# ruc-aimc-lab/GeoFormer

Measured on NVIDIA B200. Metric: pairs_per_sec_640x480, higher is better.
Workload: dtype tf32 / fp16 tensor-core operands with fp32 accumulation (fp32 residual stream, fp16 intermediates), split-fp16 similarity, f16 backbone activations

## Files before the change

### geoformer_b200/_lib.py

```python
from __future__ import annotations

import ctypes
import os
from ctypes import c_char_p, c_float, c_int, c_int64, c_void_p

HERE = os.path.dirname(os.path.abspath(__file__))
LIB_PATH = os.path.join(HERE, "libgeoformer_sm100.so")

P, I, L, F = c_void_p, c_int, c_int64, c_float

SIGNATURES = {
    "gf_abi_version": (I, []),
    "gf_last_error": (c_char_p, []),
    "gf_init": (I, [I]),
    "gf_launch_count": (L, []),
    "gf_linear_tf32": (I, [P, P, P, P, L, I, I, I, I, I, P, P, I, P, P, P, P, P]),
    "gf_linear_ref": (I, [P, P, P, P, L, I, I, I, I, I, P, P, I, P, P, P, P, P]),
    "gf_conv3x3_f16": (I, [P, P, P, P, P, I, I, I, I, I, I, I, P]),
    "gf_conv_f16": (I, [P, P, P, P, P, I, I, I, I, I, I, I, I, I, P]),
    "gf_stem_conv7x7_f16": (I, [P, P, P, P, I, I, I, P]),
    "gf_upsample_add_f16": (I, [P, P, P, I, I, I, I, I, I, P]),
    "gf_conv_ref": (I, [P, P, P, P, P, I, I, I, I, I, I, I, I, P]),
    "gf_upsample_add_ref": (I, [P, P, P, I, I, I, I, I, I, P]),
    "gf_add_posenc": (I, [P, P, P, I, L, I, P]),
    "gf_linattn_partial_floats": (L, [I, I, I, I]),
    "gf_linear_mixed": (I, [P, P, P, P, I, I, L, I, I, I, I, I, P, P, I, P, P, P, P, P]),
    "gf_fine_layer": (I, [P, P, P, P, P, P, P, P, L, P]),
    "gf_linattn_reduce_f16": (I, [P, I, P, I, I, I, I, I, P, P, P, P]),
    "gf_linattn_apply_f16": (I, [P, I, P, P, P, I, I, I, I, I, P]),
    "gf_linattn_window_f16": (I, [P, I, P, I, P, I, P, L, I, I, I, P]),
    "gf_linattn_reduce": (I, [P, I, P, I, I, I, I, I, P, P, P, P]),
    "gf_linattn_apply": (I, [P, I, P, P, P, I, I, I, I, I, P]),
    "gf_linattn_window": (I, [P, I, P, I, P, I, P, L, I, I, I, P]),
    "gf_full_attention": (I, [P, I, P, I, P, I, P, I, I, I, I, I, P]),
    "gf_dense_kv_h16": (I, [P, I, P, I, I, I, I, I, I, P, P, P, P]),
    "gf_full_attention_tc": (I, [P, I, P, P, P, P, I, I, I, I, I, I, P]),
    "gf_full_attention_window": (I, [P, I, P, I, P, I, P, L, I, I, I, P]),
    "gf_full_attention_window_f16": (I, [P, I, P, I, P, I, P, L, I, I, I, P]),
    "gf_pack_split_f16": (I, [P, P, L, I, F, I, P]),
    "gf_similarity_f16x3": (I, [P, P, P, I, I, I, I, F, P]),
    "gf_similarity_ref": (I, [P, P, P, I, I, I, I, F, F, P]),
    "gf_dual_softmax_workspace_floats": (L, [I, I, I]),
    "gf_dual_softmax_stats": (I, [P, I, I, I, P, P, P, P, P, P]),
    "gf_dual_softmax_conf": (I, [P, I, I, I, P, P, P, P, P, P, P]),
    "gf_conf_row_col_max": (I, [P, I, I, I, P, P, P]),
    "gf_mnn_select": (I, [P, I, I, I, F, I, I, I, I, I, P, P, P, P, P]),
    "gf_coarse_match_fused_workspace_bytes": (L, [I, I, I]),
    "gf_coarse_match_fused": (I, [P, P, I, I, I, I, F, F, I, I, I, I, I, P, P, P, P]),
    "gf_coarse_match_fused_pass": (I, [P, P, I, I, I, I, F, P, I, P]),
    "gf_compact_coarse": (I, [P, P, I, I, I, I, F, P, P, P, P, P, P, P, P, L, P]),
# ... 72 lines not shown
```

### geoformer_b200/csrc/fine_layer.cu

```cuda
#include "common.cuh"
#include "ptx.cuh"

#include <cuda_fp16.h>

#include <atomic>
#include <cstdlib>

namespace gf {
extern std::atomic<int64_t> g_launches;

namespace fl {
constexpr int C = 128, TOK = 25, WIN = 5, ROWS = TOK * WIN, HEADS = 8, D = 16;
constexpr int BLK = 16384;
constexpr int NBLK = 30;
constexpr int STAGES = 3;
constexpr int R1 = 0, R2 = 65536, R3 = 131072;
constexpr int R3_BYTES = 32768;
constexpr int RING = R3 + R3_BYTES;
constexpr int BARS = RING + STAGES * BLK;
constexpr int LNX = BARS + 256;
constexpr int SMEM_BYTES = LNX + 8192 + 1024;
constexpr int EPI_WARPS = 16, THREADS = 64 + 32 * EPI_WARPS;
constexpr int D0 = 0, D1 = 384, D2 = 0, D3 = 384;

struct Params {
  const float* x;
  float* y;
  const float* gamma1; const float* beta1; const float* gamma2; const float* beta2;
  int64_t rows;
  int tiles;
  int cross;
  int debug;
};

__device__ __forceinline__ float ex2f(float x) { float y; asm("ex2.approx.ftz.f32 %0, %1;" : "=f"(y) : "f"(x)); return y; }
__device__ __forceinline__ float elu_plus1(float v) { return v > 0.f ? v + 1.f : ex2f(v * 1.4426950408889634f); }
__device__ __forceinline__ uint32_t pack2(float a, float b) {
  const __half2 h = __floats2half2_rn(a, b);
  return *reinterpret_cast<const uint32_t*>(&h);
}
__device__ __forceinline__ void epi_sync() { asm volatile("bar.sync 1, 512;" ::: "memory"); }

__device__ __forceinline__ void ldsm_x4(uint32_t (&r)[4], uint32_t addr) {
  asm volatile("ldmatrix.sync.aligned.m8n8.x4.shared.b16 {%0, %1, %2, %3}, [%4];"
               : "=r"(r[0]), "=r"(r[1]), "=r"(r[2]), "=r"(r[3]) : "r"(addr));
}
__device__ __forceinline__ void ldsm_x4_trans(uint32_t (&r)[4], uint32_t addr) {
  asm volatile("ldmatrix.sync.aligned.m8n8.x4.trans.shared.b16 {%0, %1, %2, %3}, [%4];"
               : "=r"(r[0]), "=r"(r[1]), "=r"(r[2]), "=r"(r[3]) : "r"(addr));
}
__device__ __forceinline__ void mma16816(float (&d)[4], const uint32_t (&a)[4], uint32_t b0, uint32_t b1) {
  asm volatile("mma.sync.aligned.m16n8k16.row.col.f32.f16.f16.f32 {%0, %1, %2, %3}, {%4, %5, %6, %7}, {%8, %9}, {%0, %1, %2, %3};"
               : "+f"(d[0]), "+f"(d[1]), "+f"(d[2]), "+f"(d[3]) : "r"(a[0]), "r"(a[1]), "r"(a[2]), "r"(a[3]), "r"(b0), "r"(b1));
}

__device__ __forceinline__ void row_stats32(const float (&v)[32], float2* lnx, int part, int r, float& mean, float& rstd) {
  float s = 0.f, ss = 0.f;
#pragma unroll
  for (int j = 0; j < 32; ++j) { s += v[j]; ss = fmaf(v[j], v[j], ss); }
  lnx[part * 128 + r] = make_float2(s, ss);
  epi_sync();
  const float2 p0 = lnx[r], p1 = lnx[128 + r], p2 = lnx[256 + r], p3 = lnx[384 + r];
  const float ts = (p0.x + p1.x) + (p2.x + p3.x), tss = (p0.y + p1.y) + (p2.y + p3.y);
  mean = ts * (1.f / 128.f);
  const float var = fmaxf(tss * (1.f / 128.f) - mean * mean, 0.f);
  rstd = rsqrtf(var + 1e-5f);
}
__device__ __forceinline__ void normalize32(float (&v)[32], float mean, float rstd, const float* __restrict__ gamma,
                                            const float* __restrict__ beta) {
#pragma unroll
  for (int j = 0; j < 8; ++j) {
    const float4 g4 = __ldg(reinterpret_cast<const float4*>(gamma) + j);
    const float4 b4 = __ldg(reinterpret_cast<const float4*>(beta) + j);
    v[4 * j] = (v[4 * j] - mean) * rstd * g4.x + b4.x;
    v[4 * j + 1] = (v[4 * j + 1] - mean) * rstd * g4.y + b4.y;
    v[4 * j + 2] = (v[4 * j + 2] - mean) * rstd * g4.z + b4.z;
    v[4 * j + 3] = (v[4 * j + 3] - mean) * rstd * g4.w + b4.w;
  }
}
__device__ __forceinline__ void warp_arrive(uint64_t* bar, int lane) {
  ptx::fence_proxy_async();
  ptx::tc_fence_before();
  __syncwarp();
  if (lane == 0) ptx::mbar_arrive(bar);
}

__global__ void __launch_bounds__(THREADS, 1)
fine_layer_kernel(const __grid_constant__ CUtensorMap tmX, const __grid_constant__ CUtensorMap tmS,
                  const __grid_constant__ CUtensorMap tmW, const Params p) {
  extern __shared__ uint8_t smem_raw[];
  uint8_t* smem = reinterpret_cast<uint8_t*>((reinterpret_cast<uintptr_t>(smem_raw) + 1023) & ~uintptr_t(1023));
  uint64_t* full_bar = reinterpret_cast<uint64_t*>(smem + BARS);
  uint64_t* empty_bar = full_bar + STAGES;
  uint64_t* x_full = empty_bar + STAGES;
  uint64_t* s_full = x_full + 1;
  uint64_t* d_full = s_full + 1;
  uint64_t* a_full = d_full + 4;
  uint64_t* d0_free = a_full + 3;
  uint64_t* r1_free = d0_free + 1;
  uint64_t* r2_free = r1_free + 1;
  uint32_t* tmem_slot = reinterpret_cast<uint32_t*>(r2_free + 1);

  const int warp = threadIdx.x >> 5, lane = threadIdx.x & 31;

  if (warp == 0 && lane == 0) { ptx::prefetch_tmap(&tmX); ptx::prefetch_tmap(&tmS); ptx::prefetch_tmap(&tmW); }
  if (warp == 1) {
    if (lane == 0) {
      for (int i = 0; i < STAGES; ++i) { ptx::mbar_init(&full_bar[i], 1); ptx::mbar_init(&empty_bar[i], 1); }
      ptx::mbar_init(x_full, 1);
      ptx::mbar_init(s_full, 1);
      for (int i = 0; i < 4; ++i) ptx::mbar_init(&d_full[i], 1);
      for (int i = 0; i < 3; ++i) ptx::mbar_init(&a_full[i], EPI_WARPS);
      ptx::mbar_init(d0_free, 1);
      ptx::mbar_init(r1_free, 1);
      ptx::mbar_init(r2_free, 1);
      ptx::fence_barrier_init();
    }
    __syncwarp();
    ptx::tmem_alloc(tmem_slot, 512);
  }
  ptx::tc_fence_before();
  __syncthreads();
  ptx::tc_fence_after();
  const uint32_t tmem_base = *tmem_slot;

  if (warp == 0) {
    if (lane == 0) {
      int stage = 0; uint32_t phase = 0;
      auto weights = [&](int b0, int b1) {
        for (int b = b0; b < b1; ++b) {
          ptx::mbar_wait(&empty_bar[stage], phase ^ 1);
          ptx::mbar_expect_tx(&full_bar[stage], BLK);
          ptx::tma_load_3d(smem + RING + stage * BLK, &tmW, &full_bar[stage], 0, b * 128, 0);
          if (++stage == STAGES) { stage = 0; phase ^= 1; }
        }
      };
      auto load_x = [&](int t) {
        ptx::mbar_expect_tx(x_full, 4 * BLK);
        for (int kb = 0; kb < 4; ++kb) ptx::tma_load_3d(smem + R1 + kb * BLK, &tmX, x_full, kb * 32, t * ROWS, 0);
      };
      auto load_src = [&](int t) {
        ptx::mbar_expect_tx(s_full, 4 * BLK);
        for (int kb = 0; kb < 4; ++kb) ptx::tma_load_3d(smem + R2 + kb * BLK, &tmS, s_full, kb * 32, t * ROWS, 0);
      };
      load_x(blockIdx.x);
      if (p.cross) load_src(blockIdx.x);
      weights(0, 12);
      int it = 0;
      for (int t = blockIdx.x; t < p.tiles; t += gridDim.x, ++it) {
        const int tn = t + gridDim.x;
        const bool next = tn < p.tiles;
        weights(12, 20);
        if (next) { ptx::mbar_wait(r1_free, it & 1); load_x(tn); }
        weights(20, 30);
        if (next) {
          weights(0, 4);
          if (p.cross) { ptx::mbar_wait(r2_free, it & 1); load_src(tn); }
          weights(4, 12);
        }
      }
    }
  } else if (warp == 1) {
    {
      constexpr uint32_t id_tf32 = ptx::umma_idesc(2, 128, 128);
      constexpr uint32_t id_f16 = ptx::umma_idesc(0, 128, 128);
      const uint32_t smem0 = __shfl_sync(0xffffffffu, ptx::smem_addr(smem), 0);
      const uint32_t tb = __shfl_sync(0xffffffffu, tmem_base, 0);
      const uint32_t s_r1 = smem0 + R1, s_r2 = smem0 + R2, s_r3 = smem0 + R3, s_ring = smem0 + RING;
      const uint32_t bar0 = smem0 + BARS;
      auto bar_addr = [&](const uint64_t* b) -> uint32_t { return bar0 + (uint32_t)((const uint8_t*)b - (const uint8_t*)full_bar); };
      int stage = 0; uint32_t phase = 0;
      auto step = [&](int kind, uint32_t a_addr, uint32_t d_col, bool first) {
        ptx::mbar_wait(&full_bar[stage], phase);
        ptx::tc_fence_after();
        const uint32_t a_lo = ptx::umma_desc_lo(a_addr), b_lo = ptx::umma_desc_lo(s_ring + stage * BLK);
        if (ptx::elect_one()) {
          if (kind == 0) {
#pragma unroll
            for (int k = 0; k < 4; ++k) ptx::umma_lo<0>(tb + d_col, a_lo + 2 * k, b_lo + 2 * k, ptx::kDescHiSw128, id_tf32, (first && k == 0) ? 0u : 1u);
          } else {
#pragma unroll
            for (int k = 0; k < 4; ++k) ptx::umma_lo<1>(tb + d_col, a_lo + 2 * k, b_lo + 2 * k, ptx::kDescHiSw128, id_f16, (first && k == 0) ? 0u : 1u);
          }
          ptx::umma_commit_addr(bar_addr(&empty_bar[stage]));
        }
        if (++stage == STAGES) { stage = 0; phase ^= 1; }
      };
      auto commit = [&](const uint64_t* b) { if (ptx::elect_one()) ptx::umma_commit_addr(bar_addr(b)); };
      auto gemm0 = [&](int i) {
        ptx::mbar_wait(x_full, i & 1);
        ptx::tc_fence_after();
        for (int kb = 0; kb < 4; ++kb) step(0, s_r1 + kb * BLK, D0, kb == 0);
        if (p.cross) { ptx::mbar_wait(s_full, i & 1); ptx::tc_fence_after(); }
        const uint32_t a0 = p.cross ? s_r2 : s_r1;
        for (int nc = 1; nc < 3; ++nc)
          for (int kb = 0; kb < 4; ++kb) step(0, a0 + kb * BLK, D0 + nc * 128, kb == 0);
        commit(&d_full[0]);
      };
      gemm0(0);
      int it = 0;
      for (int t = blockIdx.x; t < p.tiles; t += gridDim.x, ++it) {
        const uint32_t par = it & 1;
        ptx::mbar_wait(d0_free, par);
        ptx::tc_fence_after();
        for (int nc = 0; nc < 2; ++nc)
          for (int kb = 0; kb < 4; ++kb) step(0, s_r1 + kb * BLK, D2 + nc * 128, kb == 0);
        commit(r1_free);
        ptx::mbar_wait(&a_full[0], par);
        ptx::tc_fence_after();
        for (int kb = 0; kb < 2; ++kb) step(1, s_r3 + kb * BLK, D1, kb == 0);
        commit(&d_full[1]);
        ptx::mbar_wait(&a_full[1], par);
        ptx::tc_fence_after();
        for (int nc = 0; nc < 2; ++nc)
          for (int kb = 0; kb < 2; ++kb) step(1, s_r2 + 2 * BLK + kb * BLK, D2 + nc * 128, false);
        commit(&d_full[2]);
        ptx::mbar_wait(&a_full[2], par);
        ptx::tc_fence_after();
        for (int kb = 0; kb < 4; ++kb) step(1, s_r2 + kb * BLK, D3, kb == 0);
        commit(&d_full[3]);
        commit(r2_free);
        if (t + (int)gridDim.x < p.tiles) gemm0(it + 1);
      }
    }
  } else {
    const int quad = warp & 3;
    const int part = (warp - 2) >> 2;
    const int r = quad * 32 + lane;
    const int et = threadIdx.x - 64;
    const int ew = warp - 2;
    const uint32_t t_lane = tmem_base + (uint32_t(quad * 32) << 16);
    uint8_t* r2 = smem + R2;
    uint8_t* r3 = smem + R3;
    float2* lnx = reinterpret_cast<float2*>(smem + LNX);
    const int sw7 = r & 7;
    const int g = lane >> 2, tq = lane & 3;
    const int lrow = lane & 7, lmat = lane >> 3;
    int it = 0;
    for (int t = blockIdx.x; t < p.tiles; t += gridDim.x, ++it) {
      const uint32_t par = it & 1;
      const int64_t row0 = (int64_t)t * ROWS;
      ptx::mbar_wait(&d_full[0], par);
      ptx::tc_fence_after();
      {
        float va[32], vb[32];
        ptx::tmem_ld_32x32(t_lane + D0 + 32 * part, va);
        ptx::tmem_ld_wait();
        ptx::tmem_ld_32x32(t_lane + D0 + 32 * (4 + part), vb);
        uint4 u[4];
#pragma unroll
        for (int j = 0; j < 32; ++j) va[j] = elu_plus1(va[j]);
#pragma unroll
        for (int j = 0; j < 4; ++j) {
          u[j].x = pack2(va[8 * j], va[8 * j + 1]); u[j].y = pack2(va[8 * j + 2], va[8 * j + 3]);
          u[j].z = pack2(va[8 * j + 4], va[8 * j + 5]); u[j].w = pack2(va[8 * j + 6], va[8 * j + 7]);
        }
        {
          uint8_t* dst = r3 + (part >> 1) * BLK + r * 128;
#pragma unroll
          for (int j = 0; j < 4; ++j) *reinterpret_cast<uint4*>(dst + ((((part & 1) * 4 + j) ^ sw7) << 4)) = u[j];
        }
        ptx::tmem_ld_wait();
        ptx::tmem_ld_32x32(t_lane + D0 + 32 * (8 + part), va);
#pragma unroll
        for (int j = 0; j < 32; ++j) vb[j] = elu_plus1(vb[j]);
#pragma unroll
        for (int j = 0; j < 4; ++j) {
          u[j].x = pack2(vb[8 * j], vb[8 * j + 1]); u[j].y = pack2(vb[8 * j + 2], vb[8 * j + 3]);
          u[j].z = pack2(vb[8 * j + 4], vb[8 * j + 5]); u[j].w = pack2(vb[8 * j + 6], vb[8 * j + 7]);
        }
        {
          uint8_t* dst = r2 + r * 256;
#pragma unroll
          for (int j = 0; j < 4; ++j) *reinterpret_cast<uint4*>(dst + (((part * 4 + j) ^ (r & 15)) << 4)) = u[j];
        }
        ptx::tmem_ld_wait();
#pragma unroll
        for (int j = 0; j < 4; ++j) {
          u[j].x = pack2(va[8 * j], va[8 * j + 1]); u[j].y = pack2(va[8 * j + 2], va[8 * j + 3]);
          u[j].z = pack2(va[8 * j + 4], va[8 * j + 5]); u[j].w = pack2(va[8 * j + 6], va[8 * j + 7]);
        }
        {
          uint8_t* dst = r2 + 32768 + r * 256;
#pragma unroll
          for (int j = 0; j < 4; ++j) *reinterpret_cast<uint4*>(dst + (((part * 4 + j) ^ (r & 15)) << 4)) = u[j];
        }
      }
      ptx::tc_fence_before();
      epi_sync();
      if (et == 0) ptx::mbar_arrive(d0_free);
      if (!(p.debug & 2)) {
        const uint32_t k16 = ptx::smem_addr(r2), v16 = k16 + 32768, q16 = ptx::smem_addr(r3);
#pragma unroll 1
        for (int pair = ew; pair < WIN * HEADS; pair += EPI_WARPS) {
          const int w = pair >> 3, h = pair & 7;
          float cv[2][4] = {{0.f, 0.f, 0.f, 0.f}, {0.f, 0.f, 0.f, 0.f}}, co[2][4] = {{0.f, 0.f, 0.f, 0.f}, {0.f, 0.f, 0.f, 0.f}};
#pragma unroll
          for (int ks = 0; ks < 2; ++ks) {
            const int tok0 = TOK * w + 16 * ks;
            uint32_t a[4], b[4];
            const int wlast = TOK * w + TOK - 1;
            const int arow = min(tok0 + lrow + ((lmat >> 1) << 3), wlast), achunk = 2 * h + (lmat & 1);
            ldsm_x4_trans(a, v16 + arow * 256 + ((achunk ^ (arow & 15)) << 4));
            const int brow = min(tok0 + lrow + ((lmat & 1) << 3), wlast), bchunk = 2 * h + (lmat >> 1);
            ldsm_x4_trans(b, k16 + brow * 256 + ((bchunk ^ (brow & 15)) << 4));
            uint32_t o0 = (g == 0) ? 0x3C003C00u : 0u, o2 = o0;
            if (ks == 1) {
              if (tq == 0) { a[2] &= 0xFFFFu; a[3] &= 0xFFFFu; o2 &= 0xFFFFu; } else { a[2] = 0u; a[3] = 0u; o2 = 0u; }
            }
            const uint32_t ao[4] = {o0, 0u, o2, 0u};
            mma16816(cv[0], a, b[0], b[1]); mma16816(cv[1], a, b[2], b[3]);
            mma16816(co[0], ao, b[0], b[1]); mma16816(co[1], ao, b[2], b[3]);
          }
// ... 5 lines not shown
            const int tok0 = TOK * w + 16 * mt;
            uint32_t aq[4];
            const int qrow = min(tok0 + lrow + ((lmat & 1) << 3), TOK * w + TOK - 1), qchunk = (h & 3) * 2 + (lmat >> 1);
            ldsm_x4(aq, q16 + (h >> 2) * BLK + qrow * 128 + ((qchunk ^ (qrow & 7)) << 4));
            float o0[4] = {0.f, 0.f, 0.f, 0.f}, o1[4] = {0.f, 0.f, 0.f, 0.f}, dn[4] = {0.f, 0.f, 0.f, 0.f};
            mma16816(o0, aq, bq[0][0], bq[0][1]);
            mma16816(o1, aq, bq[1][0], bq[1][1]);
            mma16816(dn, aq, bq[2][0], bq[2][1]);
            const float z_lo = 1.f / (__shfl_sync(0xffffffffu, dn[0], lane & ~3) + 1e-6f);
            const float z_hi = 1.f / (__shfl_sync(0xffffffffu, dn[2], lane & ~3) + 1e-6f);
            const int row_lo = tok0 + g, row_hi = row_lo + 8;
            __syncwarp();
            uint8_t* blk = r3 + (h >> 2) * BLK;
            const int c0 = (h & 3) * 2;
            *reinterpret_cast<uint32_t*>(blk + row_lo * 128 + ((c0 ^ (row_lo & 7)) << 4) + 4 * tq) = pack2(o0[0] * z_lo, o0[1] * z_lo);
            *reinterpret_cast<uint32_t*>(blk + row_lo * 128 + (((c0 + 1) ^ (row_lo & 7)) << 4) + 4 * tq) = pack2(o1[0] * z_lo, o1[1] * z_lo);
            if (mt == 0 || g == 0) {
              *reinterpret_cast<uint32_t*>(blk + row_hi * 128 + ((c0 ^ (row_hi & 7)) << 4) + 4 * tq) = pack2(o0[2] * z_hi, o0[3] * z_hi);
              *reinterpret_cast<uint32_t*>(blk + row_hi * 128 + (((c0 + 1) ^ (row_hi & 7)) << 4) + 4 * tq) = pack2(o1[2] * z_hi, o1[3] * z_hi);
            }
          }
        }
      }
      warp_arrive(&a_full[0], lane);
      ptx::mbar_wait(&d_full[1], par);
      ptx::tc_fence_after();
      {
        float v[32];
        ptx::tmem_ld_32x32(t_lane + D1 + 32 * part, v);
        ptx::tmem_ld_wait();
        float mean, rstd;
        row_stats32(v, lnx, part, r, mean, rstd);
        if (!(p.debug & 4)) {
          normalize32(v, mean, rstd, p.gamma1 + 32 * part, p.beta1 + 32 * part);
          uint8_t* dst = r2 + 2 * BLK + (part >> 1) * BLK + r * 128;
#pragma unroll
          for (int j = 0; j < 4; ++j) {
            uint4 u;
            u.x = pack2(v[8 * j], v[8 * j + 1]); u.y = pack2(v[8 * j + 2], v[8 * j + 3]);
            u.z = pack2(v[8 * j + 4], v[8 * j + 5]); u.w = pack2(v[8 * j + 6], v[8 * j + 7]);
            *reinterpret_cast<uint4*>(dst + ((((part & 1) * 4 + j) ^ sw7) << 4)) = u;
          }
        }
      }
      warp_arrive(&a_full[1], lane);
      ptx::mbar_wait(&d_full[2], par);
      ptx::tc_fence_after();
      {
        float va[32], vb[32];
        ptx::tmem_ld_32x32(t_lane + D2 + 32 * part, va);
        ptx::tmem_ld_32x32(t_lane + D2 + 32 * (4 + part), vb);
        ptx::tmem_ld_wait();
        if (!(p.debug & 4)) {
#pragma unroll
          for (int q = 0; q < 2; ++q) {
            const int c = part + 4 * q;
            const float* v = q ? vb : va;
            uint8_t* dst = r2 + (c >> 1) * BLK + r * 128;
#pragma unroll
            for (int j = 0; j < 4; ++j) {
              uint4 u;
              u.x = pack2(fmaxf(v[8 * j], 0.f), fmaxf(v[8 * j + 1], 0.f)); u.y = pack2(fmaxf(v[8 * j + 2], 0.f), fmaxf(v[8 * j + 3], 0.f));
              u.z = pack2(fmaxf(v[8 * j + 4], 0.f), fmaxf(v[8 * j + 5], 0.f)); u.w = pack2(fmaxf(v[8 * j + 6], 0.f), fmaxf(v[8 * j + 7], 0.f));
              *reinterpret_cast<uint4*>(dst + ((((c & 1) * 4 + j) ^ sw7) << 4)) = u;
            }
          }
        }
      }
      warp_arrive(&a_full[2], lane);
      uint8_t* box = r3 + ew * 2048;
      const int64_t grow0 = row0 + quad * 32;
      const int trow = lane >> 2, tch = lane & 3;
      float4 xr[4];
#pragma unroll
      for (int i = 0; i < 4; ++i) {
        const int rr = 8 * i + trow;
        xr[i] = make_float4(0.f, 0.f, 0.f, 0.f);
        if (quad * 32 + rr < ROWS && grow0 + rr < p.rows)
          xr[i] = __ldg(reinterpret_cast<const float4*>(p.x + (grow0 + rr) * C + 32 * part) + tch);
      }
      ptx::mbar_wait(&d_full[3], par);
      ptx::tc_fence_after();
      {
        float v[32];
        ptx::tmem_ld_32x32(t_lane + D3 + 32 * part, v);
        ptx::tmem_ld_wait();
        ptx::tc_fence_before();
        float mean, rstd;
        row_stats32(v, lnx + 512, part, r, mean, rstd);
        if (!(p.debug & 4)) {
          normalize32(v, mean, rstd, p.gamma2 + 32 * part, p.beta2 + 32 * part);
#pragma unroll
          for (int c = 0; c < 2; ++c) {
#pragma unroll
            for (int j = 0; j < 4; ++j)
              *reinterpret_cast<float4*>(box + lane * 64 + ((j ^ ((lane >> 1) & 3)) << 4)) =
                  make_float4(v[16 * c + 4 * j], v[16 * c + 4 * j + 1], v[16 * c + 4 * j + 2], v[16 * c + 4 * j + 3]);
            __syncwarp();
            float4 xn[4];
#pragma unroll
            for (int i = 0; i < 4; ++i) {
              const int rr = 8 * i + trow;
              const bool live = quad * 32 + rr < ROWS && grow0 + rr < p.rows;
              if (c == 0) {
                xn[i] = make_float4(0.f, 0.f, 0.f, 0.f);
                if (live) xn[i] = __ldg(reinterpret_cast<const float4*>(p.x + (grow0 + rr) * C + 32 * part + 16) + tch);
              }
              const float4 y4 = *reinterpret_cast<const float4*>(box + rr * 64 + ((tch ^ ((rr >> 1) & 3)) << 4));
              if (live)
                *(reinterpret_cast<float4*>(p.y + (grow0 + rr) * C + 32 * part + 16 * c) + tch) =
                    make_float4(y4.x + xr[i].x, y4.y + xr[i].y, y4.z + xr[i].z, y4.w + xr[i].w);
            }
            if (c == 0) {
#pragma unroll
              for (int i = 0; i < 4; ++i) xr[i] = xn[i];
            }
            __syncwarp();
          }
        }
      }
      epi_sync();
    }
  }

  ptx::tc_fence_before();
  __syncthreads();
  if (warp == 1) {
    ptx::tc_fence_after();
    ptx::tmem_dealloc(tmem_base, 512);
  }
}

}
}

using namespace gf;

extern "C" int gf_fine_layer(const float* x, const float* src, const void* wpack, const float* gamma1, const float* beta1,
                             const float* gamma2, const float* beta2, float* y, int64_t windows, gf_stream_t stream) {
  if (windows < 0 || !x || !src || !wpack || !y || y == x || y == src) return gf_set_error(GF_ERR_ARG, "gf_fine_layer: bad arguments");
  if (windows == 0) return GF_OK;
  const int64_t rows = windows * fl::TOK;
  if (rows > 0x7fffff00LL) return gf_set_error(GF_ERR_ARG, "gf_fine_layer: too many rows");
  CUtensorMap tx, ts, tw;
  int rc;
  if ((rc = make_tmap(&tx, x, 4, fl::C, rows, 1, fl::C, 0, 128))) return rc;
  if ((rc = make_tmap(&ts, src, 4, fl::C, rows, 1, fl::C, 0, 128))) return rc;
  if ((rc = make_tmap(&tw, wpack, 4, 32, (int64_t)fl::NBLK * 128, 1, 32, 0, 128))) return rc;
  fl::Params p{};
  p.x = x; p.y = y; p.gamma1 = gamma1; p.beta1 = beta1; p.gamma2 = gamma2; p.beta2 = beta2;
  p.rows = rows; p.tiles = (int)((windows + fl::WIN - 1) / fl::WIN); p.cross = (src != x) ? 1 : 0;
  { const char* dbg = getenv("GF_FL_DEBUG"); p.debug = dbg ? atoi(dbg) : 0; }
  GF_SMEM_OPTIN(fl::fine_layer_kernel, fl::SMEM_BYTES);
  const int grid = p.tiles < num_sms() ? p.tiles : num_sms();
  fl::fine_layer_kernel<<<grid, fl::THREADS, fl::SMEM_BYTES, (cudaStream_t)stream>>>(tx, ts, tw, p);
  g_launches++;
  GF_CHECK_LAUNCH();
  return GF_OK;
}
```

### geoformer_b200/ops.py

```python
from __future__ import annotations

import os
import threading
from typing import Optional, Tuple

import torch

from . import _lib

EPI_RELU, EPI_TANH, EPI_ELU1, EPI_LN = 1, 2, 4, 8

_LINEAR_IMPL = "tf32"
_SIM_IMPL = "f16x3"
_ATTN_IMPL = "tf32"
_ACT16 = os.environ.get("GF_ACT16", "1") != "0"


def act16() -> bool:
    return _ACT16 and _LINEAR_IMPL == "tf32"


def set_precision(linear: Optional[str] = None, similarity: Optional[str] = None,
                  attention: Optional[str] = None, activations: Optional[str] = None) -> None:
    global _LINEAR_IMPL, _SIM_IMPL, _ATTN_IMPL, _ACT16
# ... 308 lines not shown
    _call("gf_full_attention", q.data_ptr(), ldq, k.data_ptr(), ldk, v.data_ptr(), ldv, out.data_ptr(), n, l, s, heads, dim,
          _stream())
    return out


def full_attention_window(q: torch.Tensor, ldq: int, k: torch.Tensor, ldk: int, v: torch.Tensor, ldv: int, n_windows: int,
                          tokens: int, heads: int, dim: int) -> torch.Tensor:
    assert q.dtype == k.dtype == v.dtype
    out = torch.empty((n_windows * tokens, heads * dim), device=q.device, dtype=torch.float32)
    _call("gf_full_attention_window" + ("_f16" if q.dtype == torch.float16 else ""), q.data_ptr(), ldq, k.data_ptr(), ldk,
          v.data_ptr(), ldv, out.data_ptr(), n_windows, tokens, heads, dim, _stream())
    return out


def fine_layer_fused(x: torch.Tensor, src: torch.Tensor, wpack: torch.Tensor, n1w, n1b, n2w, n2b) -> torch.Tensor:
    _chk(x); _chk(src)
    m, t, c = x.shape
    assert (t, c) == (25, 128) and src.shape == x.shape and x.is_contiguous() and src.is_contiguous()
    assert wpack.dtype == torch.uint8 and wpack.shape == (30, 128, 128) and wpack.is_contiguous()
    y = torch.empty_like(x)
    _call("gf_fine_layer", x.data_ptr(), src.data_ptr(), wpack.data_ptr(), n1w.data_ptr(), n1b.data_ptr(), n2w.data_ptr(),
          n2b.data_ptr(), y.data_ptr(), m, _stream(), tag="[cross]" if src.data_ptr() != x.data_ptr() else "[self]")
    return y


def similarity(f0: torch.Tensor, f1: torch.Tensor, temperature: float, impl: Optional[str] = None) -> torch.Tensor:
    _chk(f0); _chk(f1)
    n, l, c = f0.shape
    s = f1.shape[1]
    assert f0.is_contiguous() and f1.is_contiguous()
    sim = torch.empty((n, l, s), device=f0.device, dtype=torch.float32)
    in_scale = 1.0 / c ** 0.5
    if (impl or _SIM_IMPL) == "f16x3":
        a3 = torch.empty((n, l, 3 * c), device=f0.device, dtype=torch.float16)
        b3 = torch.empty((n, s, 3 * c), device=f0.device, dtype=torch.float16)
        _call("gf_pack_split_f16", f0.data_ptr(), a3.data_ptr(), n * l, c, in_scale, 0, _stream())
        _call("gf_pack_split_f16", f1.data_ptr(), b3.data_ptr(), n * s, c, in_scale, 1, _stream())
        _call("gf_similarity_f16x3", a3.data_ptr(), b3.data_ptr(), sim.data_ptr(), n, l, s, 3 * c,
              1.0 / temperature, _stream())
    else:
        _call("gf_similarity_ref", f0.data_ptr(), f1.data_ptr(), sim.data_ptr(), n, l, s, c, in_scale,
                  1.0 / temperature, _stream())
    return sim


def dual_softmax_(sim: torch.Tensor) -> Tuple[torch.Tensor, torch.Tensor, torch.Tensor]:
# ... 212 lines not shown
```

### include/geoformer_b200.h

```cpp
#ifndef GEOFORMER_B200_H_
#define GEOFORMER_B200_H_

#include <stdint.h>

#ifdef __cplusplus
extern "C" {
#endif

#define GF_ABI_VERSION 1

#define GF_OK 0
#define GF_ERR_ARG (-1)
#define GF_ERR_LAUNCH (-2)
#define GF_ERR_DRIVER (-3)
#define GF_ERR_DEVICE (-4)

#define GF_EPI_RELU 1
#define GF_EPI_TANH 2
#define GF_EPI_ELU1 4
#define GF_EPI_LN 8

typedef void* gf_stream_t;

int gf_abi_version(void);
// ... 90 lines not shown
                        gf_stream_t stream);
int gf_masked_softmax_rows(float* x, int heads, int n, int l, int s_pad, const int* cnt_per_sample, gf_stream_t stream);
int gf_gather_anchor_kv_f16(const float* q, int ldq, const float* k, int ldk, const float* v, int ldv, int n, int l,
                            int heads, int dim, const int* anchor_idx, const int* anchor_cnt, int anchor_cap, int s_pad,
                            void* q16, void* kg, void* vt, gf_stream_t stream);
int gf_gather_anchor_kv_h16(const void* k, int ldk, const void* v, int ldv, int n, int l, int heads, int dim,
                            const int* anchor_idx, const int* anchor_cnt, int anchor_cap, int s_pad, void* kg, void* vt,
                            gf_stream_t stream);
int gf_geo_self_attention_tc(const void* q16, int ldq, const void* kg, const void* vt, float* out, int n, int l,
                             int heads, int dim, int s_pad, const int* anchor_cnt, gf_stream_t stream);
int gf_gemm_tf32_batched(const float* A, int64_t lda, int64_t a_batch_stride, const float* B, int64_t ldb,
                         int64_t b_batch_stride, float* Y, int64_t ldy, int64_t y_batch_stride, int M, int N, int K,
                         int batches, float out_scale, gf_stream_t stream);

int gf_geo_cross_attention(const float* q, int ldq, const float* kproj, int ldk, const float* vproj, int ldv,
                           float* out, int n, int l, int s, int heads, int dim, const int* widx, int window2,
                           gf_stream_t stream);
int gf_geo_cross_attention_f16(const void* q, int ldq, const void* kproj, int ldk, const void* vproj, int ldv, void* out,
                               int n, int l, int s, int heads, int dim, const int* widx, int window2, gf_stream_t stream);
int gf_select_rows(float* dst, const float* src, const int* flag, int n, int64_t l, int c, gf_stream_t stream);

int gf_fine_layer(const float* x, const float* src, const void* wpack, const float* gamma1, const float* beta1,
                  const float* gamma2, const float* beta2, float* y, int64_t windows, gf_stream_t stream);
int gf_fine_gather(const float* fine_nhwc, int hf, int wf, int c, const int64_t* b_ids, const int64_t* tok_ids,
                   int64_t m, int wc, int stride, int window, float* out, gf_stream_t stream);
int gf_fine_gather_f16(const void* fine_nhwc, int hf, int wf, int c, const int64_t* b_ids, const int64_t* tok_ids,
                        int64_t m, int wc, int stride, int window, float* out, gf_stream_t stream);
int gf_fine_gather_f16_f16(const void* fine_nhwc, int hf, int wf, int c, const int64_t* b_ids, const int64_t* tok_ids,
                            int64_t m, int wc, int stride, int window, void* out, gf_stream_t stream);
int gf_gather_rows(const float* feat, int64_t l, int c, const int64_t* b_ids, const int64_t* tok_ids, int64_t m,
                   float* out, gf_stream_t stream);
int gf_fine_match(const float* f0, const float* f1, int64_t m, int ww, int c, float temperature, float thr,
                  int* sel, int* fi, int* fj, float* fconf, float* fine_matrix, gf_stream_t stream);
int gf_compact_fine(const int* sel, const int* fi, const int* fj, const float* fconf, const float* mkpts0_c,
                    const float* mkpts1_c, const int64_t* b_ids, int64_t m, int window, float coarse_scale,
                    float c2f_scale, float fine_scale, float* mkpts0_f, float* mkpts1_f, float* mconf,
                    int64_t* m_bids, int* total, gf_stream_t stream);

int gf_resize_gray_u8(const void* src, int ho, int wo, float* dst, int ht, int wt, gf_stream_t stream);

int64_t gf_ransac_workspace_bytes(int n, int hyps);
int gf_ransac_homography(const float* k0, const float* k1, const int64_t* b_ids, const int* counts, int64_t m, int n,
                         int hyps, float thr, unsigned seed, int scale, int l0, int w0c, int l1, int w1c,
                         void* workspace, float* hmat, float* hinv, int* has_h, int* inlier, int* map0, int* map1,
                         int* anchor_idx0, int* anchor_cnt0, int* anchor_idx1, int* anchor_cnt1, int cap,
                         gf_stream_t stream);
// ... 11 lines not shown
```

Before: 486.8.

## Split fine-layer GEMM commits to overlap epilogue with MMA, add trace path

The fine transformer layer kernel now commits its GEMMs in partial chunks (first D0 chunk, low half of D2, first K-half of D3), guarded by new mbarriers, so epilogue warps can start converting outputs while the tensor core finishes the rest. In self mode the weight and chunk order is changed so the K/V chunks are ready first. The layernorm row-stat barriers become per-quad named barriers instead of a full 512-thread sync, and the final residual write drops the staging box and trailing sync in favour of direct per-row float4 stores. An optional templated clock64 trace variant and its Python entry point are added for profiling; the extra barriers and reordering add synchronisation complexity and risk of hazards.

```diff
diff --git a/geoformer_b200/_lib.py b/geoformer_b200/_lib.py
--- a/geoformer_b200/_lib.py
+++ b/geoformer_b200/_lib.py
@@ -26,6 +26,7 @@
     "gf_linattn_partial_floats": (L, [I, I, I, I]),
     "gf_linear_mixed": (I, [P, P, P, P, I, I, L, I, I, I, I, I, P, P, I, P, P, P, P, P]),
     "gf_fine_layer": (I, [P, P, P, P, P, P, P, P, L, P]),
+    "gf_fine_layer_trace": (I, [P, P, P, P, P, P, P, P, L, P, I, P]),
     "gf_linattn_reduce_f16": (I, [P, I, P, I, I, I, I, I, P, P, P, P]),
     "gf_linattn_apply_f16": (I, [P, I, P, P, P, I, I, I, I, I, P]),
     "gf_linattn_window_f16": (I, [P, I, P, I, P, I, P, L, I, I, I, P]),
diff --git a/geoformer_b200/csrc/fine_layer.cu b/geoformer_b200/csrc/fine_layer.cu
--- a/geoformer_b200/csrc/fine_layer.cu
+++ b/geoformer_b200/csrc/fine_layer.cu
@@ -31,7 +31,21 @@
   int tiles;
   int cross;
   int debug;
+  uint64_t* trace;
+  int trace_tiles;
 };
+
+enum TraceEvent {
+  M_G2X, M_G1, M_G2M, M_G3, M_G3_DONE, M_G0N, M_G0N_DONE,
+  E_D0, E_E0A, E_E0B, E_D1, E_E1, E_D2, E_E2, E_D3, E_E3,
+  P_R1_WAIT, P_R1_DONE, P_R2_WAIT, P_R2_DONE, P_RING_STALL,
+  E_D0_ALL, E_D2_HALF, E_E2_HALF,
+  TRACE_EVENTS = 24
+};
+template <bool TRACE>
+__device__ __forceinline__ void trace_at(const Params& p, int it, int ev) {
+  if (TRACE && it < p.trace_tiles) p.trace[((size_t)blockIdx.x * p.trace_tiles + it) * TRACE_EVENTS + ev] = clock64();
+}
 
 __device__ __forceinline__ float ex2f(float x) { float y; asm("ex2.approx.ftz.f32 %0, %1;" : "=f"(y) : "f"(x)); return y; }
 __device__ __forceinline__ float elu_plus1(float v) { return v > 0.f ? v + 1.f : ex2f(v * 1.4426950408889634f); }
@@ -54,12 +68,15 @@
                : "+f"(d[0]), "+f"(d[1]), "+f"(d[2]), "+f"(d[3]) : "r"(a[0]), "r"(a[1]), "r"(a[2]), "r"(a[3]), "r"(b0), "r"(b1));
 }
 
-__device__ __forceinline__ void row_stats32(const float (&v)[32], float2* lnx, int part, int r, float& mean, float& rstd) {
+__device__ __forceinline__ void quad_sync(int quad) { asm volatile("bar.sync %0, 128;" :: "r"(2 + quad) : "memory"); }
+
+__device__ __forceinline__ void row_stats32(const float (&v)[32], float2* lnx, int part, int quad, int r, float& mean,
+                                            float& rstd) {
   float s = 0.f, ss = 0.f;
 #pragma unroll
   for (int j = 0; j < 32; ++j) { s += v[j]; ss = fmaf(v[j], v[j], ss); }
   lnx[part * 128 + r] = make_float2(s, ss);
-  epi_sync();
+  quad_sync(quad);
   const float2 p0 = lnx[r], p1 = lnx[128 + r], p2 = lnx[256 + r], p3 = lnx[384 + r];
   const float ts = (p0.x + p1.x) + (p2.x + p3.x), tss = (p0.y + p1.y) + (p2.y + p3.y);
   mean = ts * (1.f / 128.f);
@@ -85,6 +102,7 @@
   if (lane == 0) ptx::mbar_arrive(bar);
 }
 
+template <bool TRACE>
 __global__ void __launch_bounds__(THREADS, 1)
 fine_layer_kernel(const __grid_constant__ CUtensorMap tmX, const __grid_constant__ CUtensorMap tmS,
                   const __grid_constant__ CUtensorMap tmW, const Params p) {
@@ -99,7 +117,10 @@
   uint64_t* d0_free = a_full + 3;
   uint64_t* r1_free = d0_free + 1;
   uint64_t* r2_free = r1_free + 1;
-  uint32_t* tmem_slot = reinterpret_cast<uint32_t*>(r2_free + 1);
+  uint64_t* d2_lo = r2_free + 1;
+  uint64_t* a2_lo = d2_lo + 1;
+  uint64_t* d0_part = a2_lo + 1;
+  uint32_t* tmem_slot = reinterpret_cast<uint32_t*>(d0_part + 1);
 
   const int warp = threadIdx.x >> 5, lane = threadIdx.x & 31;
 
@@ -114,6 +135,9 @@
       ptx::mbar_init(d0_free, 1);
       ptx::mbar_init(r1_free, 1);
       ptx::mbar_init(r2_free, 1);
+      ptx::mbar_init(d2_lo, 1);
+      ptx::mbar_init(a2_lo, EPI_WARPS);
+      ptx::mbar_init(d0_part, 1);
       ptx::fence_barrier_init();
     }
     __syncwarp();
@@ -127,9 +151,16 @@
   if (warp == 0) {
     if (lane == 0) {
       int stage = 0; uint32_t phase = 0;
+      uint64_t stall = 0;
       auto weights = [&](int b0, int b1) {
         for (int b = b0; b < b1; ++b) {
-          ptx::mbar_wait(&empty_bar[stage], phase ^ 1);
+          if (TRACE) {
+            const uint64_t c0 = clock64();
+            ptx::mbar_wait(&empty_bar[stage], phase ^ 1);
+            stall += clock64() - c0;
+          } else {
+            ptx::mbar_wait(&empty_bar[stage], phase ^ 1);
+          }
           ptx::mbar_expect_tx(&full_bar[stage], BLK);
           ptx::tma_load_3d(smem + RING + stage * BLK, &tmW, &full_bar[stage], 0, b * 128, 0);
           if (++stage == STAGES) { stage = 0; phase ^= 1; }
@@ -145,19 +176,31 @@
       };
       load_x(blockIdx.x);
       if (p.cross) load_src(blockIdx.x);
-      weights(0, 12);
+      if (p.cross) weights(0, 12); else { weights(4, 12); weights(0, 4); }
       int it = 0;
       for (int t = blockIdx.x; t < p.tiles; t += gridDim.x, ++it) {
         const int tn = t + gridDim.x;
         const bool next = tn < p.tiles;
         weights(12, 20);
-        if (next) { ptx::mbar_wait(r1_free, it & 1); load_x(tn); }
+        if (next) {
+          trace_at<TRACE>(p, it, P_R1_WAIT);
+          ptx::mbar_wait(r1_free, it & 1);
+          trace_at<TRACE>(p, it, P_R1_DONE);
+          load_x(tn);
+        }
         weights(20, 30);
-        if (next) {
+        if (next && p.cross) {
           weights(0, 4);
-          if (p.cross) { ptx::mbar_wait(r2_free, it & 1); load_src(tn); }
+          trace_at<TRACE>(p, it, P_R2_WAIT);
+          ptx::mbar_wait(r2_free, it & 1);
+          trace_at<TRACE>(p, it, P_R2_DONE);
+          load_src(tn);
           weights(4, 12);
-        }
+        } else if (next) {
+          weights(4, 12);
+          weights(0, 4);
+        }
+        if (TRACE && it < p.trace_tiles) { p.trace[((size_t)blockIdx.x * p.trace_tiles + it) * TRACE_EVENTS + P_RING_STALL] = stall; stall = 0; }
       }
     }
   } else if (warp == 1) {
@@ -190,11 +233,21 @@
       auto gemm0 = [&](int i) {
         ptx::mbar_wait(x_full, i & 1);
         ptx::tc_fence_after();
-        for (int kb = 0; kb < 4; ++kb) step(0, s_r1 + kb * BLK, D0, kb == 0);
-        if (p.cross) { ptx::mbar_wait(s_full, i & 1); ptx::tc_fence_after(); }
-        const uint32_t a0 = p.cross ? s_r2 : s_r1;
-        for (int nc = 1; nc < 3; ++nc)
+        if (lane == 0 && i > 0) trace_at<TRACE>(p, i - 1, M_G0N);
+        auto chunk = [&](int nc, uint32_t a0) {
           for (int kb = 0; kb < 4; ++kb) step(0, a0 + kb * BLK, D0 + nc * 128, kb == 0);
+        };
+        if (p.cross) {
+          chunk(0, s_r1);
+          commit(d0_part);
+          ptx::mbar_wait(s_full, i & 1);
+          ptx::tc_fence_after();
+          chunk(1, s_r2); chunk(2, s_r2);
+        } else {
+          chunk(1, s_r1); chunk(2, s_r1);
+          commit(d0_part);
+          chunk(0, s_r1);
+        }
         commit(&d_full[0]);
       };
       gemm0(0);
@@ -203,24 +256,36 @@
         const uint32_t par = it & 1;
         ptx::mbar_wait(d0_free, par);
         ptx::tc_fence_after();
+        if (lane == 0) trace_at<TRACE>(p, it, M_G2X);
         for (int nc = 0; nc < 2; ++nc)
           for (int kb = 0; kb < 4; ++kb) step(0, s_r1 + kb * BLK, D2 + nc * 128, kb == 0);
         commit(r1_free);
         ptx::mbar_wait(&a_full[0], par);
         ptx::tc_fence_after();
+        if (lane == 0) trace_at<TRACE>(p, it, M_G1);
         for (int kb = 0; kb < 2; ++kb) step(1, s_r3 + kb * BLK, D1, kb == 0);
         commit(&d_full[1]);
         ptx::mbar_wait(&a_full[1], par);
         ptx::tc_fence_after();
-        for (int nc = 0; nc < 2; ++nc)
+        if (lane == 0) trace_at<TRACE>(p, it, M_G2M);
+        for (int nc = 0; nc < 2; ++nc) {
           for (int kb = 0; kb < 2; ++kb) step(1, s_r2 + 2 * BLK + kb * BLK, D2 + nc * 128, false);
-        commit(&d_full[2]);
+          commit(nc ? &d_full[2] : d2_lo);
+        }
+        ptx::mbar_wait(a2_lo, par);
+        ptx::tc_fence_after();
+        if (lane == 0) trace_at<TRACE>(p, it, M_G3);
+        for (int kb = 0; kb < 2; ++kb) step(1, s_r2 + kb * BLK, D3, kb == 0);
         ptx::mbar_wait(&a_full[2], par);
         ptx::tc_fence_after();
-        for (int kb = 0; kb < 4; ++kb) step(1, s_r2 + kb * BLK, D3, kb == 0);
+        for (int kb = 2; kb < 4; ++kb) step(1, s_r2 + kb * BLK, D3, false);
         commit(&d_full[3]);
         commit(r2_free);
-        if (t + (int)gridDim.x < p.tiles) gemm0(it + 1);
+        if (lane == 0) trace_at<TRACE>(p, it, M_G3_DONE);
+        if (t + (int)gridDim.x < p.tiles) {
+          gemm0(it + 1);
+          if (lane == 0) trace_at<TRACE>(p, it, M_G0N_DONE);
+        }
       }
     }
   } else {
@@ -240,55 +305,59 @@
     for (int t = blockIdx.x; t < p.tiles; t += gridDim.x, ++it) {
       const uint32_t par = it & 1;
       const int64_t row0 = (int64_t)t * ROWS;
-      ptx::mbar_wait(&d_full[0], par);
-      ptx::tc_fence_after();
       {
+        auto store_q = [&](float (&v)[32]) {
+#pragma unroll
+          for (int j = 0; j < 32; ++j) v[j] = elu_plus1(v[j]);
+          uint8_t* dst = r3 + (part >> 1) * BLK + r * 128;
+#pragma unroll
+          for (int j = 0; j < 4; ++j) {
+            uint4 u;
+            u.x = pack2(v[8 * j], v[8 * j + 1]); u.y = pack2(v[8 * j + 2], v[8 * j + 3]);
+            u.z = pack2(v[8 * j + 4], v[8 * j + 5]); u.w = pack2(v[8 * j + 6], v[8 * j + 7]);
+            *reinterpret_cast<uint4*>(dst + ((((part & 1) * 4 + j) ^ sw7) << 4)) = u;
+          }
+        };
+        auto store_kv = [&](float (&v)[32], int off, bool elu) {
+          if (elu) {
+#pragma unroll
+            for (int j = 0; j < 32; ++j) v[j] = elu_plus1(v[j]);
+          }
+          uint8_t* dst = r2 + off + r * 256;
+#pragma unroll
+          for (int j = 0; j < 4; ++j) {
+            uint4 u;
+            u.x = pack2(v[8 * j], v[8 * j + 1]); u.y = pack2(v[8 * j + 2], v[8 * j + 3]);
+            u.z = pack2(v[8 * j + 4], v[8 * j + 5]); u.w = pack2(v[8 * j + 6], v[8 * j + 7]);
+            *reinterpret_cast<uint4*>(dst + (((part * 4 + j) ^ (r & 15)) << 4)) = u;
+          }
+        };
         float va[32], vb[32];
-        ptx::tmem_ld_32x32(t_lane + D0 + 32 * part, va);
-        ptx::tmem_ld_wait();
-        ptx::tmem_ld_32x32(t_lane + D0 + 32 * (4 + part), vb);
-        uint4 u[4];
-#pragma unroll
-        for (int j = 0; j < 32; ++j) va[j] = elu_plus1(va[j]);
-#pragma unroll
-        for (int j = 0; j < 4; ++j) {
-          u[j].x = pack2(va[8 * j], va[8 * j + 1]); u[j].y = pack2(va[8 * j + 2], va[8 * j + 3]);
-          u[j].z = pack2(va[8 * j + 4], va[8 * j + 5]); u[j].w = pack2(va[8 * j + 6], va[8 * j + 7]);
-        }
-        {
-          uint8_t* dst = r3 + (part >> 1) * BLK + r * 128;
-#pragma unroll
-          for (int j = 0; j < 4; ++j) *reinterpret_cast<uint4*>(dst + ((((part & 1) * 4 + j) ^ sw7) << 4)) = u[j];
-        }
-        ptx::tmem_ld_wait();
-        ptx::tmem_ld_32x32(t_lane + D0 + 32 * (8 + part), va);
-#pragma unroll
-        for (int j = 0; j < 32; ++j) vb[j] = elu_plus1(vb[j]);
-#pragma unroll
-        for (int j = 0; j < 4; ++j) {
-          u[j].x = pack2(vb[8 * j], vb[8 * j + 1]); u[j].y = pack2(vb[8 * j + 2], vb[8 * j + 3]);
-          u[j].z = pack2(vb[8 * j + 4], vb[8 * j + 5]); u[j].w = pack2(vb[8 * j + 6], vb[8 * j + 7]);
-        }
-        {
-          uint8_t* dst = r2 + r * 256;
-#pragma unroll
-          for (int j = 0; j < 4; ++j) *reinterpret_cast<uint4*>(dst + (((part * 4 + j) ^ (r & 15)) << 4)) = u[j];
-        }
-        ptx::tmem_ld_wait();
-#pragma unroll
-        for (int j = 0; j < 4; ++j) {
-          u[j].x = pack2(va[8 * j], va[8 * j + 1]); u[j].y = pack2(va[8 * j + 2], va[8 * j + 3]);
-          u[j].z = pack2(va[8 * j + 4], va[8 * j + 5]); u[j].w = pack2(va[8 * j + 6], va[8 * j + 7]);
-        }
-        {
-          uint8_t* dst = r2 + 32768 + r * 256;
-#pragma unroll
-          for (int j = 0; j < 4; ++j) *reinterpret_cast<uint4*>(dst + (((part * 4 + j) ^ (r & 15)) << 4)) = u[j];
-        }
+        auto kv = [&]() {
+          ptx::tmem_ld_32x32(t_lane + D0 + 32 * (4 + part), va);
+          ptx::tmem_ld_wait();
+          ptx::tmem_ld_32x32(t_lane + D0 + 32 * (8 + part), vb);
+          store_kv(va, 0, true);
+          ptx::tmem_ld_wait();
+          store_kv(vb, 32768, false);
+        };
+        auto q = [&]() {
+          ptx::tmem_ld_32x32(t_lane + D0 + 32 * part, va);
+          ptx::tmem_ld_wait();
+          store_q(va);
+        };
+        ptx::mbar_wait(d0_part, par);
+        ptx::tc_fence_after();
+        if (et == 0) trace_at<TRACE>(p, it, E_D0);
+        if (p.cross) q(); else kv();
+        ptx::mbar_wait(&d_full[0], par);
+        ptx::tc_fence_after();
+        if (et == 0) trace_at<TRACE>(p, it, E_D0_ALL);
+        if (p.cross) kv(); else q();
       }
       ptx::tc_fence_before();
       epi_sync();
-      if (et == 0) ptx::mbar_arrive(d0_free);
+      if (et == 0) { ptx::mbar_arrive(d0_free); trace_at<TRACE>(p, it, E_E0A); }
       if (!(p.debug & 2)) {
         const uint32_t k16 = ptx::smem_addr(r2), v16 = k16 + 32768, q16 = ptx::smem_addr(r3);
 #pragma unroll 1
@@ -340,15 +409,17 @@
           }
         }
       }
+      if (et == 0) trace_at<TRACE>(p, it, E_E0B);
       warp_arrive(&a_full[0], lane);
       ptx::mbar_wait(&d_full[1], par);
       ptx::tc_fence_after();
+      if (et == 0) trace_at<TRACE>(p, it, E_D1);
       {
         float v[32];
         ptx::tmem_ld_32x32(t_lane + D1 + 32 * part, v);
         ptx::tmem_ld_wait();
         float mean, rstd;
-        row_stats32(v, lnx, part, r, mean, rstd);
+        row_stats32(v, lnx, part, quad, r, mean, rstd);
         if (!(p.debug & 4)) {
           normalize32(v, mean, rstd, p.gamma1 + 32 * part, p.beta1 + 32 * part);
           uint8_t* dst = r2 + 2 * BLK + (part >> 1) * BLK + r * 128;
@@ -362,82 +433,58 @@
         }
       }
       warp_arrive(&a_full[1], lane);
-      ptx::mbar_wait(&d_full[2], par);
-      ptx::tc_fence_after();
-      {
-        float va[32], vb[32];
-        ptx::tmem_ld_32x32(t_lane + D2 + 32 * part, va);
-        ptx::tmem_ld_32x32(t_lane + D2 + 32 * (4 + part), vb);
+      if (et == 0) trace_at<TRACE>(p, it, E_E1);
+#pragma unroll 1
+      for (int q = 0; q < 2; ++q) {
+        ptx::mbar_wait(q ? &d_full[2] : d2_lo, par);
+        ptx::tc_fence_after();
+        if (et == 0) trace_at<TRACE>(p, it, q ? E_D2 : E_D2_HALF);
+        const int c = part + 4 * q;
+        float v[32];
+        ptx::tmem_ld_32x32(t_lane + D2 + 32 * c, v);
         ptx::tmem_ld_wait();
         if (!(p.debug & 4)) {
-#pragma unroll
-          for (int q = 0; q < 2; ++q) {
-            const int c = part + 4 * q;
-            const float* v = q ? vb : va;
-            uint8_t* dst = r2 + (c >> 1) * BLK + r * 128;
-#pragma unroll
-            for (int j = 0; j < 4; ++j) {
-              uint4 u;
-              u.x = pack2(fmaxf(v[8 * j], 0.f), fmaxf(v[8 * j + 1], 0.f)); u.y = pack2(fmaxf(v[8 * j + 2], 0.f), fmaxf(v[8 * j + 3], 0.f));
-              u.z = pack2(fmaxf(v[8 * j + 4], 0.f), fmaxf(v[8 * j + 5], 0.f)); u.w = pack2(fmaxf(v[8 * j + 6], 0.f), fmaxf(v[8 * j + 7], 0.f));
-              *reinterpret_cast<uint4*>(dst + ((((c & 1) * 4 + j) ^ sw7) << 4)) = u;
-            }
-          }
-        }
-      }
-      warp_arrive(&a_full[2], lane);
-      uint8_t* box = r3 + ew * 2048;
-      const int64_t grow0 = row0 + quad * 32;
-      const int trow = lane >> 2, tch = lane & 3;
-      float4 xr[4];
-#pragma unroll
-      for (int i = 0; i < 4; ++i) {
-        const int rr = 8 * i + trow;
-        xr[i] = make_float4(0.f, 0.f, 0.f, 0.f);
-        if (quad * 32 + rr < ROWS && grow0 + rr < p.rows)
-          xr[i] = __ldg(reinterpret_cast<const float4*>(p.x + (grow0 + rr) * C + 32 * part) + tch);
-      }
+          uint8_t* dst = r2 + (c >> 1) * BLK + r * 128;
+#pragma unroll
+          for (int j = 0; j < 4; ++j) {
+            uint4 u;
+            u.x = pack2(fmaxf(v[8 * j], 0.f), fmaxf(v[8 * j + 1], 0.f)); u.y = pack2(fmaxf(v[8 * j + 2], 0.f), fmaxf(v[8 * j + 3], 0.f));
+            u.z = pack2(fmaxf(v[8 * j + 4], 0.f), fmaxf(v[8 * j + 5], 0.f)); u.w = pack2(fmaxf(v[8 * j + 6], 0.f), fmaxf(v[8 * j + 7], 0.f));
+            *reinterpret_cast<uint4*>(dst + ((((c & 1) * 4 + j) ^ sw7) << 4)) = u;
+          }
+        }
+        warp_arrive(q ? &a_full[2] : a2_lo, lane);
+        if (et == 0) trace_at<TRACE>(p, it, q ? E_E2 : E_E2_HALF);
+      }
+      const int64_t grow = row0 + r;
+      const bool live = r < ROWS && grow < p.rows;
+      const float4* xrow = reinterpret_cast<const float4*>(p.x + grow * C + 32 * part);
+      float4* yrow = reinterpret_cast<float4*>(p.y + grow * C + 32 * part);
+      float4 xr[8];
+#pragma unroll
+      for (int j = 0; j < 4; ++j) xr[j] = live ? __ldg(xrow + j) : make_float4(0.f, 0.f, 0.f, 0.f);
       ptx::mbar_wait(&d_full[3], par);
       ptx::tc_fence_after();
+      if (et == 0) trace_at<TRACE>(p, it, E_D3);
       {
         float v[32];
         ptx::tmem_ld_32x32(t_lane + D3 + 32 * part, v);
+#pragma unroll
+        for (int j = 4; j < 8; ++j) xr[j] = live ? __ldg(xrow + j) : make_float4(0.f, 0.f, 0.f, 0.f);
         ptx::tmem_ld_wait();
         ptx::tc_fence_before();
         float mean, rstd;
-        row_stats32(v, lnx + 512, part, r, mean, rstd);
+        row_stats32(v, lnx + 512, part, quad, r, mean, rstd);
         if (!(p.debug & 4)) {
           normalize32(v, mean, rstd, p.gamma2 + 32 * part, p.beta2 + 32 * part);
-#pragma unroll
-          for (int c = 0; c < 2; ++c) {
-#pragma unroll
-            for (int j = 0; j < 4; ++j)
-              *reinterpret_cast<float4*>(box + lane * 64 + ((j ^ ((lane >> 1) & 3)) << 4)) =
-                  make_float4(v[16 * c + 4 * j], v[16 * c + 4 * j + 1], v[16 * c + 4 * j + 2], v[16 * c + 4 * j + 3]);
-            __syncwarp();
-            float4 xn[4];
-#pragma unroll
-            for (int i = 0; i < 4; ++i) {
-              const int rr = 8 * i + trow;
-              const bool live = quad * 32 + rr < ROWS && grow0 + rr < p.rows;
-              if (c == 0) {
-                xn[i] = make_float4(0.f, 0.f, 0.f, 0.f);
-                if (live) xn[i] = __ldg(reinterpret_cast<const float4*>(p.x + (grow0 + rr) * C + 32 * part + 16) + tch);
-              }
-              const float4 y4 = *reinterpret_cast<const float4*>(box + rr * 64 + ((tch ^ ((rr >> 1) & 3)) << 4));
-              if (live)
-                *(reinterpret_cast<float4*>(p.y + (grow0 + rr) * C + 32 * part + 16 * c) + tch) =
-                    make_float4(y4.x + xr[i].x, y4.y + xr[i].y, y4.z + xr[i].z, y4.w + xr[i].w);
-            }
-            if (c == 0) {
-#pragma unroll
-              for (int i = 0; i < 4; ++i) xr[i] = xn[i];
-            }
-            __syncwarp();
-          }
-        }
-      }
-      epi_sync();
+          if (live) {
+#pragma unroll
+            for (int j = 0; j < 8; ++j)
+              yrow[j] = make_float4(v[4 * j] + xr[j].x, v[4 * j + 1] + xr[j].y, v[4 * j + 2] + xr[j].z, v[4 * j + 3] + xr[j].w);
+          }
+        }
+      }
+      if (et == 0) trace_at<TRACE>(p, it, E_E3);
     }
   }
 
@@ -454,8 +501,10 @@
 
 using namespace gf;
 
-extern "C" int gf_fine_layer(const float* x, const float* src, const void* wpack, const float* gamma1, const float* beta1,
-                             const float* gamma2, const float* beta2, float* y, int64_t windows, gf_stream_t stream) {
+namespace {
+int launch_fine_layer(const float* x, const float* src, const void* wpack, const float* gamma1, const float* beta1,
+                      const float* gamma2, const float* beta2, float* y, int64_t windows, uint64_t* trace, int trace_tiles,
+                      gf_stream_t stream) {
   if (windows < 0 || !x || !src || !wpack || !y || y == x || y == src) return gf_set_error(GF_ERR_ARG, "gf_fine_layer: bad arguments");
   if (windows == 0) return GF_OK;
   const int64_t rows = windows * fl::TOK;
@@ -469,10 +518,29 @@
   p.x = x; p.y = y; p.gamma1 = gamma1; p.beta1 = beta1; p.gamma2 = gamma2; p.beta2 = beta2;
   p.rows = rows; p.tiles = (int)((windows + fl::WIN - 1) / fl::WIN); p.cross = (src != x) ? 1 : 0;
   { const char* dbg = getenv("GF_FL_DEBUG"); p.debug = dbg ? atoi(dbg) : 0; }
-  GF_SMEM_OPTIN(fl::fine_layer_kernel, fl::SMEM_BYTES);
+  p.trace = trace; p.trace_tiles = trace_tiles;
   const int grid = p.tiles < num_sms() ? p.tiles : num_sms();
-  fl::fine_layer_kernel<<<grid, fl::THREADS, fl::SMEM_BYTES, (cudaStream_t)stream>>>(tx, ts, tw, p);
+  if (trace) {
+    GF_SMEM_OPTIN(fl::fine_layer_kernel<true>, fl::SMEM_BYTES);
+    fl::fine_layer_kernel<true><<<grid, fl::THREADS, fl::SMEM_BYTES, (cudaStream_t)stream>>>(tx, ts, tw, p);
+  } else {
+    GF_SMEM_OPTIN(fl::fine_layer_kernel<false>, fl::SMEM_BYTES);
+    fl::fine_layer_kernel<false><<<grid, fl::THREADS, fl::SMEM_BYTES, (cudaStream_t)stream>>>(tx, ts, tw, p);
+  }
   g_launches++;
   GF_CHECK_LAUNCH();
   return GF_OK;
 }
+}
+
+extern "C" int gf_fine_layer(const float* x, const float* src, const void* wpack, const float* gamma1, const float* beta1,
+                             const float* gamma2, const float* beta2, float* y, int64_t windows, gf_stream_t stream) {
+  return launch_fine_layer(x, src, wpack, gamma1, beta1, gamma2, beta2, y, windows, nullptr, 0, stream);
+}
+
+extern "C" int gf_fine_layer_trace(const float* x, const float* src, const void* wpack, const float* gamma1,
+                                   const float* beta1, const float* gamma2, const float* beta2, float* y, int64_t windows,
+                                   uint64_t* trace, int trace_tiles, gf_stream_t stream) {
+  if (!trace || trace_tiles < 1) return gf_set_error(GF_ERR_ARG, "gf_fine_layer_trace: bad trace buffer");
+  return launch_fine_layer(x, src, wpack, gamma1, beta1, gamma2, beta2, y, windows, trace, trace_tiles, stream);
+}
diff --git a/geoformer_b200/ops.py b/geoformer_b200/ops.py
--- a/geoformer_b200/ops.py
+++ b/geoformer_b200/ops.py
@@ -354,6 +354,19 @@
     _call("gf_fine_layer", x.data_ptr(), src.data_ptr(), wpack.data_ptr(), n1w.data_ptr(), n1b.data_ptr(), n2w.data_ptr(),
           n2b.data_ptr(), y.data_ptr(), m, _stream(), tag="[cross]" if src.data_ptr() != x.data_ptr() else "[self]")
     return y
+
+
+def fine_layer_fused_trace(x: torch.Tensor, src: torch.Tensor, wpack: torch.Tensor, n1w, n1b, n2w, n2b, trace_tiles: int):
+    _chk(x); _chk(src)
+    m, t, c = x.shape
+    assert (t, c) == (25, 128) and src.shape == x.shape and x.is_contiguous() and src.is_contiguous() and trace_tiles >= 1
+    assert wpack.dtype == torch.uint8 and wpack.shape == (30, 128, 128) and wpack.is_contiguous()
+    ctas = min((m + 4) // 5, torch.cuda.get_device_properties(x.device).multi_processor_count)
+    trace = torch.zeros((ctas, trace_tiles, 24), device=x.device, dtype=torch.int64)
+    y = torch.empty_like(x)
+    _call("gf_fine_layer_trace", x.data_ptr(), src.data_ptr(), wpack.data_ptr(), n1w.data_ptr(), n1b.data_ptr(),
+          n2w.data_ptr(), n2b.data_ptr(), y.data_ptr(), m, trace.data_ptr(), trace_tiles, _stream())
+    return y, trace
 
 
 def similarity(f0: torch.Tensor, f1: torch.Tensor, temperature: float, impl: Optional[str] = None) -> torch.Tensor:
diff --git a/include/geoformer_b200.h b/include/geoformer_b200.h
--- a/include/geoformer_b200.h
+++ b/include/geoformer_b200.h
@@ -136,6 +136,9 @@
 
 int gf_fine_layer(const float* x, const float* src, const void* wpack, const float* gamma1, const float* beta1,
                   const float* gamma2, const float* beta2, float* y, int64_t windows, gf_stream_t stream);
+int gf_fine_layer_trace(const float* x, const float* src, const void* wpack, const float* gamma1, const float* beta1,
+                        const float* gamma2, const float* beta2, float* y, int64_t windows, uint64_t* trace,
+                        int trace_tiles, gf_stream_t stream);
 int gf_fine_gather(const float* fine_nhwc, int hf, int wf, int c, const int64_t* b_ids, const int64_t* tok_ids,
                    int64_t m, int wc, int stride, int window, float* out, gf_stream_t stream);
 int gf_fine_gather_f16(const void* fine_nhwc, int hf, int wf, int c, const int64_t* b_ids, const int64_t* tok_ids,
```

Result: slower. 472.4 (median of 6 runs) (-3.0%).
